# maxjiang93/space_time_pde

Measured on AMD Instinct MI355X. Metric: query-points/sec (fwd+PDE-residual bwd), rb2d 128^3 latent, higher is better.
Workload: dtype f32; 1 GPU; BASELINE configs[1]: latent [1,32,128,128,32], 2^20 query points, RB2 (3 transport + continuity), ImNet nf=32 softplus, L1 losses, backward to ImNet + UNet3d parameters; points=1048576, parallelism=points sharded x1, unet=UNet3d(igres=(32, 128, 128), nf=16, mf=256) fwd+bwd inside the timed step

## Files before the change

include/stpde_hip.h:

```cpp
#ifndef STPDE_HIP_H
#define STPDE_HIP_H

#ifdef __cplusplus
extern "C" {
#endif

#define STPDE_OK 0
#define STPDE_E_BADARG 1
#define STPDE_E_UNSUPPORTED 2
#define STPDE_E_LAUNCH 3

#define STPDE_ACT_TANH 0
#define STPDE_ACT_RELU 1
#define STPDE_ACT_SOFTPLUS 2
#define STPDE_ACT_ELU 3
#define STPDE_ACT_SWISH 4
#define STPDE_ACT_LEAKYRELU 5

#define STPDE_XT 3
#define STPDE_PBAR_SLOTS 64

typedef struct {
  int S1;
  int S2;
  int pair0[6];
  int pair1[6];
  int act;
  float act_param;
  int combo;
  float alpha[6];
} stpde_jet_cfg;

int stpde_version(void);
int stpde_last_error(char* buf, unsigned long n);
#define STPDE_TUNE_CONV3_LDS_OFF 0
#define STPDE_TUNE_CONV3_LDS_MINBLK 1
#define STPDE_TUNE_CONV3_LDS_GX 2
#define STPDE_TUNE_CONV_WGRAD_LDS_GX 3
#define STPDE_TUNE_CONV1_WGRAD_LDS_GX 4
#define STPDE_TUNE_WGRAD_FP32_SWAP 5
#define STPDE_TUNE_COUNT 6
int stpde_tune(const char* name, int value);
int stpde_trace_enable(int on);
long stpde_trace_read(char* buf, unsigned long n);

typedef struct {
  int P, N, B, n0, n1, n2, C;
  int p_base;
  float lo_c[3], hi_c[3], cube[3];
  float alpha[6];
} stpde_gather_desc;
int stpde_lig_gather(const stpde_gather_desc* d, const float* pts, const float* latent, float* X, float* XR,
                     float* coef, int* cell, float* cw , void* stream);

typedef struct {
  int ntiles, KT, MT, first_hidden;
  stpde_jet_cfg cfg;
  int mfma_bf16;
  int packed;
  int det;
} stpde_layer_desc;
int stpde_jet_layer_fwd(const stpde_layer_desc* d, const float* in_pre, const float* X, const float* Wh_pack,
                        const float* Ws_pack, const float* tanc, const float* W0s_pack, const float* tanc0,
                        float* out_pre, const float* cw ,
// ... 10 lines not shown
int stpde_jet_tail_bwd(const stpde_jet_cfg* cfg, int ntiles, int nf16, const float* abar5, const float* const* WhT_pack,
                       const float* const* pre, float* const* abar_out, const float* cw, float* act_param_bar,
                       void* stream);

int stpde_jet_tail_bwd_p(const stpde_jet_cfg* cfg, int ntiles, int nf16, const float* abar5, const float* const* WhT_pack,
                         const float* const* pre, float* const* abar_out, const float* cw, float* act_param_bar, int packed,
                         const void* const* WhT16_pack, void* stream);

int stpde_jet_layer_bwd(const stpde_layer_desc* d, const float* abar_out, const float* WhT_pack, float* in_pre,
                        const float* X, const float* W0s_pack, const float* tanc0, float* abar0, const float* cw,
                        float* act_param_bar, const void* WhT_pack_bf16 ,
                        float* abar0_tan, const float* z0, void* stream);

int stpde_jet_layer_bwd_to(const stpde_layer_desc* d, const float* abar_out, const float* WhT_pack, const float* in_pre,
                           float* abar_in, const float* cw, float* act_param_bar, const void* WhT_pack_bf16, void* stream);

int stpde_jet_wgrad(const stpde_layer_desc* d, int SP, const float* abar_out, const float* in_pre, const float* X,
                    const float* tanc0, float* dW_aug, const float* cw, void* stream);

int stpde_jet_fc1_bwd_supported(const stpde_layer_desc* d);
int stpde_jet_fc1_bwd(const stpde_layer_desc* d, const float* abar1, const void* WhT_pack_bf16, const float* z0,
                      const float* tanc0, const float* cw, const float* X, float* abar0, float* abar0_tan, float* dW_aug,
                      float* act_param_bar, void* stream);

int stpde_lig_reduce_fwd(const stpde_jet_cfg* cfg, int S_mlp, int P, int n_out, const float* out_pre,
                         const float* coef, float* jets, long ldp, void* stream);
int stpde_lig_reduce_bwd(const stpde_jet_cfg* cfg, int S_mlp, int P, int n_out, const float* jets_bar, long ldp,
                         const float* coef, float* abar_out, void* stream);

int stpde_jet_tan0_reduce(int ntiles, int MT, const float* abar0_tan, float* dW_aug, int ldw, int det ,
                          void* stream);

typedef struct {
  int ntiles, nlayers, C, n1, n2;
  int MT[8];
  int SP[8];
  int packed[8];
  int S[8];
} stpde_xbar_desc;
int stpde_lig_xbar_scatter(const stpde_xbar_desc* d, const float* const* abar, const float* const* WsL_pack,
                           const int* cell, float* dlatent, void* stream);
int stpde_lig_xbar_rows(const stpde_xbar_desc* d, const float* const* abar, const float* const* WsL_pack,
                        float* xrows, void* stream);
int stpde_lig_dlatent_reduce(int B, int n0, int n1, int n2, int C, const float* xrows, const int* perm,
                             const int* start, float* dlatent, void* stream);

// ... 23 lines not shown
  float* abar3x;
  float* tan0;
  float* abar0;
  float* abar1x;
  float* abar0x;
  float* xrows;
  int* perm;
  int* start;
  void* sort_tmp;
  unsigned long sort_tmp_bytes;
  float* abar4x;
} stpde_lig_workspace;
#define STPDE_F_STASH 1
#define STPDE_F_VALUE_TILES 2
#define STPDE_F_FUSED_TAIL 4
#define STPDE_F_TAN0_ROWSUM 8
#define STPDE_F_DETERMINISTIC 16
#define STPDE_F_WGRAD 32
#define STPDE_F_WGRAD_FP32 64
#define STPDE_F_PHASE_A 128
#define STPDE_F_PHASE_B 256
#define STPDE_F_NO_FC1_FUSED 512
#define STPDE_F_DET 1024
int stpde_lig_imnet_jet_fwd(const stpde_imnet_plan* plan, const stpde_jet_cfg* cfg_mlp, const stpde_jet_cfg* cfg_out,
                            const stpde_gather_desc* gd, const float* pts, const float* latent,
                            const stpde_lig_workspace* ws, float* jets, long ldp, int flags, void* stream);
int stpde_lig_imnet_jet_bwd(const stpde_imnet_plan* plan, const stpde_jet_cfg* cfg_mlp, const stpde_jet_cfg* cfg_out,
                            const stpde_jet_cfg* cfg_val, const stpde_gather_desc* gd, const stpde_lig_workspace* ws,
                            const float* jets_bar, long ldp, float* dW_flat, float* dlatent, float* act_param_bar,
                            int flags, void* stream);
unsigned long stpde_lig_sort_tmp_bytes(int P, long n_nodes);
int stpde_lig_cell_sort(int P, long n_nodes, const int* cell, int* perm, int* start, void* tmp, unsigned long tmp_bytes,
                        void* stream);

typedef struct {
  int P, N, B, dim, C;
  int n[4];
  float lo_c[4], hi_c[4], cube[4];
} stpde_interp_desc;
int stpde_interp_fwd(const stpde_interp_desc* d, const float* grid, const float* pts, float* out ,
                     float* corner_values , float* weights ,
                     float* x_relative , void* stream);
int stpde_interp_bwd_grid(const stpde_interp_desc* d, const float* pts, const float* out_bar,
                          const float* corner_bar, float* dgrid, void* stream);

typedef struct {
// ... 248 lines not shown
```

space_time_pde_amd/_lib.py:

```python
import ctypes as C
import os
import subprocess
import threading

_HERE = os.path.dirname(os.path.abspath(__file__))
_CSRC = os.path.join(_HERE, "csrc")
LIB_PATH = os.environ.get("STPDE_LIB") or os.path.join(_HERE, "libstpde_hip.so")
_SOURCES = ["jet_layer.hip", "jet_layer_s00.hip", "jet_layer_s03.hip", "jet_layer_s30.hip", "jet_layer_s31.hip", "jet_layer_s32.hip", "jet_layer_s34.hip", "jet_layer_s36.hip", "jet_tail.hip", "jet_wgrad.hip", "jet_wgrad_s00.hip", "jet_wgrad_s30.hip", "jet_wgrad_s31.hip", "jet_wgrad_s32.hip", "jet_wgrad_s34.hip", "jet_wgrad_s36.hip", "jet_fc1_bwd.hip", "lig_gather_reduce.hip", "lig_pipeline.hip", "interp_nd.hip", "conv3d.hip", "conv3d_fused.hip", "optim.hip", "residual.hip", "bn.hip", "resample.hip", "sampler.hip", "sampler_median.hip", "api.cpp"]
_HIPFLAGS = ["--offload-arch=gfx950", "-O3", "-std=c++17", "-fPIC", "-ffp-contract=off", "-munsafe-fp-atomics",
             "--offload-compress"]

ABI_VERSION = 316

ACT_CODES = {"tanh": 0, "relu": 1, "softplus": 2, "elu": 3, "swish": 4, "leakyrelu": 5}
PBAR_SLOTS = 64
XT = 3


class JetCfg(C.Structure):
    _fields_ = [("S1", C.c_int), ("S2", C.c_int), ("pair0", C.c_int * 6), ("pair1", C.c_int * 6),
                ("act", C.c_int), ("act_param", C.c_float), ("combo", C.c_int), ("alpha", C.c_float * 6)]


class GatherDesc(C.Structure):
    _fields_ = [("P", C.c_int), ("N", C.c_int), ("B", C.c_int), ("n0", C.c_int), ("n1", C.c_int), ("n2", C.c_int),
                ("C", C.c_int), ("p_base", C.c_int), ("lo_c", C.c_float * 3), ("hi_c", C.c_float * 3),
                ("cube", C.c_float * 3), ("alpha", C.c_float * 6)]


class GatherNdDesc(C.Structure):
    _fields_ = [("D", C.c_int), ("P", C.c_int), ("N", C.c_int), ("B", C.c_int), ("C", C.c_int), ("p_base", C.c_int),
# ... 6 lines not shown
                ("mfma_bf16", C.c_int), ("packed", C.c_int), ("det", C.c_int)]


class XbarDesc(C.Structure):
    _fields_ = [("ntiles", C.c_int), ("nlayers", C.c_int), ("C", C.c_int), ("n1", C.c_int), ("n2", C.c_int),
                ("MT", C.c_int * 8), ("SP", C.c_int * 8), ("packed", C.c_int * 8), ("S", C.c_int * 8)]


class ImNetPlanDesc(C.Structure):
    _fields_ = [("nlayers", C.c_int), ("cin", C.c_int), ("cout", C.c_int), ("nf16", C.c_int), ("KT", C.c_int * 8),
                ("MT", C.c_int * 8), ("Wh", C.c_void_p * 8), ("WhT", C.c_void_p * 8), ("Ws", C.c_void_p * 8),
                ("WsL", C.c_void_p * 8), ("tanc", C.c_void_p * 8), ("Wh16", C.c_void_p * 8), ("WhT16", C.c_void_p * 8),
                ("mfma_bf16", C.c_int), ("packed_mask", C.c_int), ("dw_off", C.c_long * 8)]


class LigWorkspace(C.Structure):
    _fields_ = [("X", C.c_void_p), ("XR", C.c_void_p), ("coef", C.c_void_p), ("cw", C.c_void_p), ("cell", C.c_void_p),
                ("pre", C.c_void_p * 8), ("abar2x", C.c_void_p), ("abar3x", C.c_void_p), ("tan0", C.c_void_p),
                ("abar0", C.c_void_p), ("abar1x", C.c_void_p), ("abar0x", C.c_void_p), ("xrows", C.c_void_p), ("perm", C.c_void_p), ("start", C.c_void_p),
                ("sort_tmp", C.c_void_p), ("sort_tmp_bytes", C.c_ulong), ("abar4x", C.c_void_p)]


F_STASH, F_VALUE_TILES, F_FUSED_TAIL, F_TAN0_ROWSUM, F_DETERMINISTIC, F_WGRAD, F_WGRAD_FP32 = 1, 2, 4, 8, 16, 32, 64
F_PHASE_A, F_PHASE_B, F_NO_FC1_FUSED, F_DET = 128, 256, 512, 1024
LOSS_DET = 16


class Conv3dDesc(C.Structure):
    _fields_ = [("B", C.c_int), ("T", C.c_int), ("Z", C.c_int), ("X", C.c_int), ("Ci", C.c_int), ("Co", C.c_int),
                ("ksize", C.c_int), ("det", C.c_int), ("mfma_bf16", C.c_int)]


class Conv3dFusedArgs(C.Structure):
    _fields_ = [("d", Conv3dDesc), ("x", C.c_void_p), ("w_pack", C.c_void_p), ("bias", C.c_void_p), ("y", C.c_void_p),
                ("x2", C.c_void_p), ("w2_pack", C.c_void_p), ("y2", C.c_void_p), ("wo2_pack", C.c_void_p),
                ("bias2", C.c_void_p), ("in_sums", C.c_void_p), ("in_gamma", C.c_void_p), ("in_beta", C.c_void_p),
                ("in_running_mean", C.c_void_p), ("in_running_var", C.c_void_p), ("in_stat", C.c_void_p),
                ("out_sums", C.c_void_p), ("m", C.c_void_p), ("m_stat", C.c_void_p), ("m_gamma", C.c_void_p),
                ("m_beta", C.c_void_p), ("m_bsum", C.c_void_p), ("Ci2", C.c_int), ("Co2", C.c_int),
                ("in_eps", C.c_float), ("in_momentum", C.c_float)]


class ResampleDesc(C.Structure):
    _fields_ = [("B", C.c_int), ("T", C.c_int), ("Z", C.c_int), ("X", C.c_int), ("C", C.c_int), ("ft", C.c_int),
                ("fz", C.c_int), ("fx", C.c_int)]


# ... 155 lines not shown
    "stpde_lig_dlatent_reduce_nd": ([C.c_int, C.c_int, C.POINTER(C.c_int), C.c_int, _VP, _VP, _VP, _VP, _VP], C.c_int),
    "stpde_lig_coef_nd": ([C.POINTER(GatherNdDesc), _VP, _VP, _VP], C.c_int),
    "stpde_lig_reduce_nd_jet_fwd": ([C.POINTER(JetCfg), C.c_int, C.c_int, C.c_int, C.c_int, C.c_int, _VP, _VP, _VP, C.c_long,
                                     _VP], C.c_int),
    "stpde_lig_reduce_nd_jet_bwd": ([C.POINTER(JetCfg), C.c_int, C.c_int, C.c_int, C.c_int, C.c_int, _VP, C.c_long, _VP, _VP,
                                     _VP], C.c_int),
    "stpde_jet_wgrad_nd": ([C.POINTER(LayerDesc), C.c_int] + [_VP] * 6 + [C.c_int, _VP], C.c_int),
    "stpde_jet_tan0_reduce_nd": ([C.c_int, C.c_int, _VP, _VP, C.c_int, C.c_int, C.c_int, _VP], C.c_int),
    "stpde_jet_layer_fwd": ([C.POINTER(LayerDesc)] + [_VP] * 12, C.c_int),
    "stpde_jet_layer_bwd": ([C.POINTER(LayerDesc)] + [_VP] * 13, C.c_int),
    "stpde_jet_layer_bwd_to": ([C.POINTER(LayerDesc)] + [_VP] * 8, C.c_int),
    "stpde_jet_tail_fwd": ([C.POINTER(JetCfg), C.c_int, C.c_int, _VP, _VP, C.POINTER(_VP), C.POINTER(_VP), C.POINTER(_VP),
                            C.POINTER(_VP), _VP, _VP], C.c_int),
    "stpde_jet_tail_bwd": ([C.POINTER(JetCfg), C.c_int, C.c_int, _VP, C.POINTER(_VP), C.POINTER(_VP), C.POINTER(_VP), _VP,
                            _VP, _VP], C.c_int),
    "stpde_jet_tail_fwd_p": ([C.POINTER(JetCfg), C.c_int, C.c_int, _VP, _VP, C.POINTER(_VP), C.POINTER(_VP), C.POINTER(_VP),
                              C.POINTER(_VP), _VP, C.c_int, C.POINTER(_VP), _VP], C.c_int),
    "stpde_jet_tail_bwd_p": ([C.POINTER(JetCfg), C.c_int, C.c_int, _VP, C.POINTER(_VP), C.POINTER(_VP), C.POINTER(_VP), _VP,
                              _VP, C.c_int, C.POINTER(_VP), _VP], C.c_int),
    "stpde_jet_tan0_reduce": ([C.c_int, C.c_int, _VP, _VP, C.c_int, C.c_int, _VP], C.c_int),
    "stpde_jet_wgrad": ([C.POINTER(LayerDesc), C.c_int] + [_VP] * 7, C.c_int),
    "stpde_jet_fc1_bwd_supported": ([C.POINTER(LayerDesc)], C.c_int),
    "stpde_jet_fc1_bwd": ([C.POINTER(LayerDesc)] + [_VP] * 11, C.c_int),
    "stpde_lig_reduce_fwd": ([C.POINTER(JetCfg), C.c_int, C.c_int, C.c_int, _VP, _VP, _VP, C.c_long, _VP], C.c_int),
    "stpde_lig_reduce_bwd": ([C.POINTER(JetCfg), C.c_int, C.c_int, C.c_int, _VP, C.c_long, _VP, _VP, _VP], C.c_int),
    "stpde_lig_xbar_scatter": ([C.POINTER(XbarDesc), C.POINTER(_VP), C.POINTER(_VP), _VP, _VP, _VP], C.c_int),
    "stpde_lig_xbar_rows": ([C.POINTER(XbarDesc), C.POINTER(_VP), C.POINTER(_VP), _VP, _VP], C.c_int),
    "stpde_lig_dlatent_reduce": ([C.c_int] * 5 + [_VP] * 5, C.c_int),
    "stpde_lig_imnet_jet_fwd": ([C.POINTER(ImNetPlanDesc), C.POINTER(JetCfg), C.POINTER(JetCfg), C.POINTER(GatherDesc), _VP,
                                 _VP, C.POINTER(LigWorkspace), _VP, C.c_long, C.c_int, _VP], C.c_int),
    "stpde_lig_imnet_jet_bwd": ([C.POINTER(ImNetPlanDesc), C.POINTER(JetCfg), C.POINTER(JetCfg), C.POINTER(JetCfg),
                                 C.POINTER(GatherDesc), C.POINTER(LigWorkspace), _VP, C.c_long, _VP, _VP, _VP, C.c_int, _VP],
                                C.c_int),
    "stpde_lig_sort_tmp_bytes": ([C.c_int, C.c_long], C.c_ulong),
    "stpde_lig_cell_sort": ([C.c_int, C.c_long, _VP, _VP, _VP, _VP, C.c_ulong, _VP], C.c_int),
    "stpde_interp_fwd": ([C.POINTER(InterpDesc)] + [_VP] * 7, C.c_int),
    "stpde_interp_bwd_grid": ([C.POINTER(InterpDesc)] + [_VP] * 5, C.c_int),
    "stpde_conv3d_fwd": ([C.POINTER(Conv3dDesc)] + [_VP] * 5, C.c_int),
    "stpde_conv3d_wgrad": ([C.POINTER(Conv3dDesc)] + [_VP] * 4, C.c_int),
    "stpde_conv3d_wgrad_bias": ([C.POINTER(Conv3dDesc)] + [_VP] * 5, C.c_int),
    "stpde_conv3d_fused": ([C.POINTER(Conv3dFusedArgs), C.POINTER(C.c_int), _VP], C.c_int),
    "stpde_conv3d_wgrad_onload": ([C.POINTER(Conv3dDesc)] + [_VP] * 8, C.c_int),
    "stpde_residual_fwd": ([_VP, C.c_int, C.c_int, C.c_int, C.c_int, _VP, C.c_long, C.c_long, _VP, _VP, _VP], C.c_int),
    "stpde_residual_bwd": ([_VP, C.c_int, C.c_int, C.c_int, C.c_int, _VP, C.c_long, C.c_long, _VP, _VP, _VP, _VP],
                           C.c_int),
    "stpde_residual_coef_fwd": ([_VP, C.c_int, C.c_int, C.c_int, C.c_int, _VP, C.c_long, C.c_long, _VP, _VP,
# ... 46 lines not shown
                    fn.restype = restype
                if h.stpde_version() != ABI_VERSION:
                    raise RuntimeError("libstpde_hip.so at %s has ABI version %d, this package needs %d: rebuild it "
                                       "(python -c 'import __graft_entry__ as g; g.build()')"
                                       % (LIB_PATH, h.stpde_version(), ABI_VERSION))
                _lib = h
    return _lib


_EXC = {1: ValueError, 2: NotImplementedError, 3: RuntimeError}


def check(rc):
    if rc != 0:
        buf = C.create_string_buffer(512)
        lib().stpde_last_error(buf, 512)
        raise _EXC.get(rc, RuntimeError)("libstpde_hip: " + buf.value.decode())


def tune(name, value):
    prev = lib().stpde_tune(name.encode(), int(value))
    if prev < 0:
        raise KeyError(name)
    return prev


class tuned:

    def __init__(self, **kv):
        self.kv, self.prev = kv, {}

    def __enter__(self):
        for k, v in self.kv.items():
            self.prev[k] = tune(k, v)
        return self

    def __exit__(self, *exc):
        for k, v in self.prev.items():
            tune(k, v)
        return False


class dispatch_trace:

    def __enter__(self):
        lib().stpde_trace_enable(1)
        self.kernels = []
# ... 61 lines not shown
```

space_time_pde_amd/csrc/api.cpp:

```cpp
#include <hip/hip_runtime.h>

#include <cstdarg>
#include <cstdio>
#include <cstring>
#include <mutex>
#include <set>
#include <string>

#include "../../include/stpde_hip.h"

static thread_local char g_err[512] = "";

void stpde_set_error(const char* fmt, ...) {
  va_list ap;
  va_start(ap, fmt);
  vsnprintf(g_err, sizeof(g_err), fmt, ap);
  va_end(ap);
}

int stpde_check_launch(const char* what) {
  hipError_t e = hipGetLastError();
  if (e != hipSuccess) {
    stpde_set_error("%s: launch failed: %s", what, hipGetErrorString(e));
    return STPDE_E_LAUNCH;
  }
  return STPDE_OK;
}

extern "C" int stpde_version(void) { return 316; }

#include <atomic>
static const char* const g_tune_names[STPDE_TUNE_COUNT] = {"conv3_lds_off", "conv3_lds_minblk", "conv3_lds_gx", "conv_wgrad_lds_gx",
                                                           "conv1_wgrad_lds_gx", "wgrad_fp32_swap"};
static std::atomic<int> g_tune[STPDE_TUNE_COUNT];
int stpde_tune_get(int key) { return (key >= 0 && key < STPDE_TUNE_COUNT) ? g_tune[key].load(std::memory_order_relaxed) : 0; }
extern "C" int stpde_tune(const char* name, int value) {
  if (!name) return -1;
  for (int k = 0; k < STPDE_TUNE_COUNT; ++k)
    if (!strcmp(name, g_tune_names[k])) return g_tune[k].exchange(value);
  stpde_set_error("stpde_tune: unknown key '%s'", name);
  return -1;
}

extern "C" int stpde_last_error(char* buf, unsigned long n) {
  if (!buf || n == 0) return STPDE_E_BADARG;
  strncpy(buf, g_err, n - 1);
  buf[n - 1] = 0;
  return STPDE_OK;
}

int stpde_trace_on = 0;
static std::mutex g_trace_mu;
static std::set<std::string> g_trace;

void stpde_trace_note(const char* launcher, const char* kernel) {
  std::lock_guard<std::mutex> lk(g_trace_mu);
// ... 21 lines not shown
```

space_time_pde_amd/csrc/lig_pipeline.hip:

```cpp
#include <hipcub/hipcub.hpp>

#include "common.h"

namespace {

struct Seq {
  int rc = STPDE_OK;
  template <class F>
  void operator()(F&& f) {
    if (rc == STPDE_OK) rc = f();
  }
};

bool is_packed(const stpde_imnet_plan* p, int l) { return l >= 0 && ((p->packed_mask >> l) & 1); }

int packed_flags(const stpde_imnet_plan* p, int l, int writes) {
  return ((l >= 2 && is_packed(p, l - 1)) ? 1 : 0) | ((writes >= 0 && is_packed(p, writes)) ? 2 : 0) | (is_packed(p, l) ? 4 : 0);
}

stpde_layer_desc layer_desc(int ntiles, const stpde_imnet_plan* p, int l, const stpde_jet_cfg& cfg, int bf16) {
  stpde_layer_desc d{};
  d.ntiles = ntiles;
  d.KT = p->KT[l];
  d.MT = p->MT[l];
// ... 205 lines not shown
      });
      return;
    }
    seq([&] {
      return stpde_jet_layer_bwd(&d, abar[l], p->WhT[l], l > 1 ? ws->pre[l - 1] : nullptr, ws->X, p->Ws[0], p->tanc[0], abar0,
                                 ws->cw, act_param_bar, w16, (l == 1 && split0) ? ws->tan0 : nullptr, l == 1 ? z0 : nullptr,
                                 stream);
    });
  };
  const bool fc1_fused_on = [&]() -> bool {
    if (!wgrad || !split0 || (flags & STPDE_F_NO_FC1_FUSED)) return false;
    stpde_layer_desc d = layer_desc(nt, p, 1, cfg, p->mfma_bf16 ? p->mfma_bf16 : 0);
    d.packed = packed_flags(p, 1, 0);
    return p->WhT16[1] && stpde_jet_fc1_bwd_supported(&d) != 0 && abar0 != z0;
  }();
  auto fc1_fused_ok = [&]() -> bool { return fc1_fused_on; };
  auto fc1_fused = [&] {
    stpde_layer_desc d = layer_desc(nt, p, 1, cfg, p->mfma_bf16);
    d.packed = packed_flags(p, 1, 0);
    d.det = det;
    seq([&] {
      return stpde_jet_fc1_bwd(&d, abar[1], p->WhT16[1], z0, p->tanc[0], ws->cw, ws->X, abar0, ws->tan0,
                               dW_flat + aw * p->dw_off[1], act_param_bar, stream);
    });
  };
  auto dlatent_part = [&] {
    if (!dlatent) return;
    stpde_xbar_desc xd{};
    xd.ntiles = nt;
    xd.nlayers = 5;
    xd.C = p->cin;
    xd.n1 = gd->n1;
    xd.n2 = gd->n2;
    const float* ab[5];
    const float* wt[5];
    for (int l = 0; l < 5; ++l) {
      xd.MT[l] = p->MT[l];
      xd.SP[l] = l == 0 ? (split0 ? 1 : SP0) : S;
      xd.packed[l] = is_packed(p, l) ? 1 : 0;
      xd.S[l] = l == 0 ? 1 : S;
      ab[l] = l == 0 ? abar0 : abar[l];
      wt[l] = p->WsL[l];
    }
    if (!(flags & STPDE_F_DETERMINISTIC)) {
      seq([&] { return stpde_lig_xbar_scatter(&xd, ab, wt, ws->cell, dlatent, stream); });
    } else {
// ... 10 lines not shown
    if (phaseA) {
      seq([&] { return stpde_lig_reduce_bwd(cfg_out, S, gd->P, p->cout, jets_bar, ldp, ws->coef, ws->pre[NL - 1], stream); });
      if (wgrad) wgrad_l(5);
      tail_bwd();
      dgrad_l(2);
      if (fc1_fused_ok())
        fc1_fused();
      else
        dgrad_l(1);
      dlatent_part();
    }
    if (phaseB && wgrad) {
      for (int l = 4; l >= (fc1_fused_ok() ? 2 : 1); --l) wgrad_l(l);
      wgrad_0();
    }
    return seq.rc;
  }
  seq([&] { return stpde_lig_reduce_bwd(cfg_out, S, gd->P, p->cout, jets_bar, ldp, ws->coef, ws->pre[NL - 1], stream); });
  for (int l = NL - 1; l >= 1; --l) {
    if (l == 1 && fc1_fused_ok()) {
      fc1_fused();
      continue;
    }
    if (wgrad) wgrad_l(l);
    if (tail && l >= 3) {
      if (l == 5) tail_bwd();
      continue;
    }
    dgrad_l(l);
  }
  if (wgrad) wgrad_0();
  dlatent_part();
  return seq.rc;
}
```

space_time_pde_amd/lig_jet.py:

```python
import ctypes as C
import dataclasses
import math
import os
import threading

import numpy as np
import torch

from . import _lib
from ._lib import XT, GatherDesc, GatherNdDesc, ImNetPlanDesc, JetCfg, LayerDesc, LigWorkspace, XbarDesc, check, ptr, stream_ptr

_FRAG = 256
MAX_LATENT_CHANNELS = 16 * (XT - 1) + 4 - 3 - 1
MAX_AUG_FEATURES = 16 * (XT - 1) + 4
ND_VALUE_DIMS = (1, 2, 4)
ND_TRAIN_MAX_CHANNELS = 32

nd_backward = os.getenv("STPDE_ND_BACKWARD", "0").strip().lower() not in ("", "0", "false", "no", "off")


def set_nd_backward(on):
    global nd_backward
    prev, nd_backward = nd_backward, bool(on)
    return prev
# ... 300 lines not shown
    S_out: int
    pairs: list
    bf16: bool
    nsplit: int
    packed_mask: int
    B: int
    N: int
    grid_shape: tuple
    lo_c: list
    hi_c: list
    cube: list
    P_pad: int
    budget: object
    recompute: bool
    chunk: int
    need_grad: bool
    det: bool
    det_dlatent: bool
    value_tiles: bool
    tan0_rowsum: bool
    wgrad_split: bool
    fused_tail: bool
    fc1_fused: bool
    nd_backward: bool
    nd_jets: bool
    nd_jet_backward: bool
    pipeline: bool
    tail: bool
    SP0: int
    split0: bool
    mult: int

    @classmethod
    def make(cls, plan, act, act_param, first, pairs, combo, precision, grid_shape, box, budget=None, B=1, N=0,
             chunk_points=None, need_grad=True):
        precision = precision or mlp_precision
        if precision not in ("fp32", "bf16", "fp32x3"):
            raise ValueError("mlp precision must be 'fp32', 'bf16' or 'fp32x3'")
        dim = plan.dim
        if dim != 3 and precision == "bf16":
            raise NotImplementedError("dim = %d value queries run with fp32 or fp32x3 operands" % dim)
        cfg_out, S_out, ppairs = make_cfg(act, act_param, first, list(pairs), combo)
        cfg, S = cfg_out, S_out
        if act in ("relu", "leakyrelu") and ppairs:
            cfg, S, _ = make_cfg(act, act_param, True, [])
        tail = _tail_applies(fused_tail, plan.nf, cfg, cfg_out.combo)
        packed = (precision == "bf16" and packed_stash and plan.nf == 32 and S <= 6 and tail and cfg.S1 == 3 and tan0_rowsum)
        mult = (8 if S == 1 else 2) if dim == 3 else 4 * (16 >> dim)
        chunk_points = chunk_points or (DEFAULT_CHUNK if dim == 3 else (DEFAULT_CHUNK // 2) * (16 >> dim))
        P, SP0 = B * N, 1 + cfg.S1
        return cls(plan=plan, cfg=cfg, cfg_out=cfg_out, cfg_val=make_cfg(act, act_param, False, [])[0], S=S, S_out=S_out,
                   pairs=ppairs, bf16=precision in ("bf16", "fp32x3"), nsplit=3 if precision == "fp32x3" else 1,
                   packed_mask=31 if packed else 0, B=B, N=N, grid_shape=tuple(grid_shape), lo_c=box[0], hi_c=box[1],
                   cube=box[2], P_pad=P + ((-P) % mult if dim == 3 else 0),
                   budget=budget if budget is not None else memory_budget, recompute=bool(force_recompute),
                   chunk=max(mult, chunk_points // mult * mult), need_grad=bool(need_grad), det=bool(_lib.deterministic),
                   det_dlatent=bool(deterministic_dlatent), value_tiles=bool(value_tiles), tan0_rowsum=bool(tan0_rowsum),
                   wgrad_split=bool(wgrad_split), fused_tail=bool(fused_tail), fc1_fused=fc1_fused_enabled(),
                   nd_backward=bool(nd_backward), nd_jets=bool(nd_jets),
                   nd_jet_backward=bool(nd_jets and nd_jet_backward),
                   pipeline=bool(use_pipeline and profile is None and dim == 3),
                   tail=tail, SP0=SP0, split0=bool(SP0 == 4 and tan0_rowsum), mult=mult)

    def plan_chunk(self, points):
        object.__setattr__(self, "chunk", points)


def _AW(call):
    return 2 * _lib.DET_K if call.det else 1


def _dw_slice(call, dw_flat, l):
    off, mp, ka = call.plan.dw_off[l]
    return dw_flat[_AW(call) * off:_AW(call) * (off + mp * ka)]


def _layer_desc(call, ntiles, lay, cfg, first_hidden, bf16=0, packed=0):
    d = LayerDesc()
    d.ntiles, d.KT, d.MT, d.first_hidden, d.cfg = ntiles, lay["KT"], lay["MT"], int(first_hidden), cfg
    d.mfma_bf16 = int(bf16)
    d.packed = int(packed)
# ... 41 lines not shown
        if packs16:
            d.Wh16[l], d.WhT16[l] = _dp(packs16.get((l, "Wh"))), _dp(packs16.get((l, "WhT")))
        d.dw_off[l] = plan.dw_off[l][0]
    d.mfma_bf16 = call.nsplit if packs16 else 0
    d.packed_mask = call.packed_mask
    return d


def _gather_desc(call, latent, Pc, p0):
    gd = GatherDesc()
    gd.P, gd.N, gd.B = Pc, call.N, call.B
    gd.n0, gd.n1, gd.n2, gd.C = latent.shape[1], latent.shape[2], latent.shape[3], latent.shape[4]
    for k in range(3):
        gd.lo_c[k], gd.hi_c[k], gd.cube[k] = call.lo_c[k], call.hi_c[k], call.cube[k]
    gd.p_base = p0
    for k in range(6):
        gd.alpha[k] = call.cfg_out.alpha[k]
    return gd


def _flags(call, need_grad, need_wgrad=True):
    bits = ((need_grad, _lib.F_STASH), (call.value_tiles, _lib.F_VALUE_TILES), (call.fused_tail, _lib.F_FUSED_TAIL),
            (call.tan0_rowsum, _lib.F_TAN0_ROWSUM), (call.det_dlatent, _lib.F_DETERMINISTIC), (need_wgrad, _lib.F_WGRAD),
            (not call.wgrad_split, _lib.F_WGRAD_FP32), (not call.fc1_fused, _lib.F_NO_FC1_FUSED), (call.det, _lib.F_DET))
    return sum(bit for on, bit in bits if on)


def nd_tiles(P, dim):
    tp = 16 >> dim
    return (-(-P // tp) + 3) // 4 * 4


_LAYER_BUFS = tuple("buf%d" % l for l in range(1, 6))
_FWD_ORDER = {True: ("X", "cw", "coef", "cell") + _LAYER_BUFS + ("z0",),
              False: ("X", "cw", "roww", "coef", "cell", "buf1", "z0") + _LAYER_BUFS[1:]}
_BWD_ORDER = {True: ("abar2x", "abar3x", "abar1x", "abar4x", "abar0x", "tan0", "abar0"),
              False: ("abar0", "abar0x", "tan0", "abar1x", "abar4x", "abar3x", "abar2x")}
_DTYPES = dict(cell=torch.int32, perm=torch.int32, start=torch.int32, sort_tmp=torch.uint8)
SORT_TMP_PLAN_BYTES = 24


def _table(order, size):
    return [(k, size[k], _DTYPES.get(k, torch.float32)) for k in order if size.get(k) is not None]


def _chunk_tiles(call, Pc):
    return nd_tiles(Pc, call.plan.dim) if call.plan.dim != 3 else Pc // 2
# ... 186 lines not shown
    elif nd:
        with _timed("reduce_nd_bwd"):
            check(L.stpde_lig_reduce_nd_bwd(plan.dim, Pc, nt, plan.cout, C.c_void_p(jets_bar.data_ptr() + 4 * p0),
                                            jets_bar.shape[2], ptr(saved["roww"]), ptr(bufs[5]), st))
    else:
        with _timed("reduce_bwd"):
            check(L.stpde_lig_reduce_bwd(C.byref(call.cfg_out), S, Pc, plan.cout, C.c_void_p(jets_bar.data_ptr() + 4 * p0),
                                         jets_bar.shape[2], ptr(coef), ptr(bufs[5]), st))
    MT0 = plan.layers[0]["MT"]
    adj = _alloc(_backward_buffers(call, Pc), dev)
    abar0, tan0 = adj.get("abar0x", adj.get("abar0", z0)), adj.get("tan0")
    abar = {l: adj.get("abar%dx" % l, bufs[l]) for l in range(1, 6)}
    for l in range(5, 0, -1):
        lay = plan.layers[l]
        w16 = packs16.get((l, "WhT")) if packs16 else None
        d = _layer_desc(call, nt, lay, cfg, l == 1, call.nsplit if w16 is not None else 0, _pk(call, l, l - 1))
        dwg = _layer_desc(call, nt, lay, cfg, l == 1, (call.nsplit if call.wgrad_split or call.nsplit == 1 else 0)
                          if (w16 is not None and lay["MT"] >= 8) else 0, _pk(call, l, -1) & 5)
        if (l == 1 and need_wgrad and split0 and w16 is not None and abar0 is not z0
                and call.fc1_fused and L.stpde_jet_fc1_bwd_supported(C.byref(d))):
            with _timed("layer1_bwd"):
                check(L.stpde_jet_fc1_bwd(C.byref(d), ptr(abar[1]), ptr(w16), ptr(z0), ptr(pv(packs, 0, "tanc")), ptr(cw),
                                          ptr(X), ptr(abar0), ptr(tan0), ptr(_dw_slice(call, dw_flat, 1)), ptr(pbar), st))
            continue
        if need_wgrad:
            with _timed("layer%d_wgrad" % l):
                check(wgrad(dwg, S, abar[l], bufs[l - 1] if l > 1 else saved["z0"], pv(packs, 0, "tanc"),
                            _dw_slice(call, dw_flat, l), cw))
        if call.tail and l >= 3:
            if l == 5:
                arr = lambda ts: (C.c_void_p * 3)(*[t.data_ptr() for t in ts])
                pk_tail = (call.packed_mask >> 2) & 1
                w16s = (C.c_void_p * 3)(packs16[(3, "WhT")].data_ptr(), packs16[(4, "WhT")].data_ptr(), None) \
                    if pk_tail else None
                with _timed("tail_dgrad"):
                    check(L.stpde_jet_tail_bwd_p(C.byref(cfg), nt, plan.nf // 16, ptr(bufs[5]),
                                                 arr([pv(packs, k, "WhT") for k in (3, 4, 5)]),
                                                 arr([bufs[2], bufs[3], bufs[4]]), arr([abar[2], abar[3], abar[4]]),
                                                 ptr(cw), ptr(pbar), 3 if pk_tail else 0, w16s, st))
            continue
        if l > 1 and abar[l - 1] is not bufs[l - 1]:
            with _timed("layer%d_dgrad" % l):
                check(L.stpde_jet_layer_bwd_to(C.byref(d), ptr(abar[l]), ptr(pv(packs, l, "WhT")), ptr(bufs[l - 1]),
                                               ptr(abar[l - 1]), ptr(cw), ptr(pbar), ptr(w16), st))
            continue
        with _timed("layer%d_dgrad" % l):
# ... 236 lines not shown
        if type(module) is cls:
            if name == "softplus" and (module.beta != 1 or module.threshold != 20):
                return None
            if name == "elu" and module.alpha != 1.0:
                return None
            if name == "leakyrelu" and module.negative_slope != 0.01:
                return None
            return name, 0.0
    return None


deterministic_dlatent = True
value_tiles = True
tan0_rowsum = True
wgrad_split = True
packed_stash = True
fused_tail = True

force_recompute = False


def fc1_fused_enabled():
    return os.environ.get("STPDE_FC1_FUSED", "1") != "0"

DEFAULT_CHUNK = 1 << 20

mlp_precision = os.environ.get("STPDE_MLP_PRECISION", "fp32")


def set_mlp_precision(precision):
    global mlp_precision
    if precision not in ("fp32", "bf16", "fp32x3"):
        raise ValueError("mlp precision must be 'fp32', 'bf16' or 'fp32x3'")
    prev, mlp_precision = mlp_precision, precision
    return prev


_ND_VALUE_ONLY = "dim = %d queries run in HIP as value-only forward passes (no coordinate derivatives)"


def lig_jets(imnet, latent_grid, query_pts, xmin, xmax, first=True, pairs=(), chunk_points=None, combo=None,
             precision=None, memory_budget=None):
    if not (latent_grid.is_cuda and query_pts.is_cuda):
        raise RuntimeError("the HIP jet path needs CUDA/HIP tensors (no CPU fallback)")
    dim = imnet.dim
    wants_jets = bool(first or len(pairs) or combo)
# ... 72 lines not shown
```

space_time_pde_amd/train_step.py:

```python
import os

import torch
import torch.distributed as dist
import torch.nn.functional as F

from . import _lib, lig_jet
from .local_implicit_grid import query_local_implicit_grid


last_collectives = []


class _SumGradAcrossRanks(torch.autograd.Function):

    @staticmethod
    def forward(ctx, x):
        return x.view_as(x)

    @staticmethod
    def backward(ctx, g):
        hooks = lig_jet.sync_hooks
        done = hooks.get("dlatent_done") if hooks else None
        if done is None:
            g = g.contiguous()
# ... 52 lines not shown
            and not (b is not None and b.requires_grad):
        return _LossSumHip.apply(a, b, _LOSS_KIND[loss_type])
    return _LOSS_SUMS[loss_type](a, torch.zeros_like(a) if b is None else b)


def _coefficient_leaves(pde_layer):
    vals = getattr(pde_layer, "params", None) or {}
    return [vals[s.name] for s in getattr(pde_layer, "param_vars", ()) if s.name in vals and vals[s.name].requires_grad
            and vals[s.name].is_leaf]


def sharded_step(unet, imnet, pde_layer, input_grid, point_coord, point_value, n_points_global, alpha_reg=1.0,
                 alpha_pde=1.0, loss_type="l1", xmin=0.0, xmax=1.0, distributed=None, sync_unet_grads=False):
    if distributed is None:
        distributed = dist.is_available() and dist.is_initialized() and dist.get_world_size() > 1
    if loss_type not in _LOSS_SUMS:
        raise KeyError(loss_type)
    if distributed and any(t.requires_grad and not t.is_leaf for t in (getattr(pde_layer, "params", None) or {}).values()):
        raise NotImplementedError("sharded_step(distributed=True): a grad-requiring equation coefficient must be a leaf tensor "
                                  "(the gradient of a leaf behind it would not be summed over ranks)")
    prev_deferred = getattr(unet, "deferred_weight_grads", None)
    if prev_deferred is not None:
        unet.deferred_weight_grads = os.environ.get("STPDE_UNET_DEFERRED", "1") != "0"
    try:
        return _sharded_step(unet, imnet, pde_layer, input_grid, point_coord, point_value, n_points_global, alpha_reg,
                             alpha_pde, loss_type, xmin, xmax, distributed, sync_unet_grads)
    finally:
        if prev_deferred is not None:
            unet.deferred_weight_grads = prev_deferred


def _sharded_step(unet, imnet, pde_layer, input_grid, point_coord, point_value, n_points_global, alpha_reg, alpha_pde,
                  loss_type, xmin, xmax, distributed, sync_unet_grads):
    latent_grid = unet(input_grid).permute(0, 2, 3, 4, 1)
    if distributed:
        latent_grid = _SumGradAcrossRanks.apply(latent_grid)
    pde_layer.update_forward_method(lambda pts: query_local_implicit_grid(imnet, latent_grid, pts, xmin, xmax))
    overlap_sync = distributed and os.environ.get("STPDE_OVERLAP_SYNC", "1") != "0"
    lig_jet.expect_two_phase = bool(overlap_sync)
    try:
        pred, residues = pde_layer(point_coord, return_residue=True)
    finally:
        lig_jet.expect_two_phase = False
    b = point_coord.shape[0]
    reg = loss_sum(pred, point_value, loss_type) / (b * n_points_global * pred.shape[-1])
    res = list(residues.values())
    base = res[0]._base if all(r._base is not None and r._base is res[0]._base for r in res) else None
    stack = base if (base is not None and base.numel() == sum(r.numel() for r in res)) else torch.stack(res, dim=0)
    pde = loss_sum(stack, None, loss_type) / (len(res) * b * n_points_global)
    loss = alpha_reg * reg + alpha_pde * pde
# ... 178 lines not shown
```

Before: 2.523 million query-points/s.

## Fuse second hidden layer backward data-grad and weight-grad into one kernel

Adds a fused HIP kernel for the layer-2 ImNet jet backward that computes the adjoint into layer 1 (through the activation jet) and the weight gradient, including the raw-input and tangent row-sum columns, in a single pass over the tiles. The goal is to avoid reading abar2 and pre1 twice across separate backward-to and wgrad launches, and to save a launch. It is switched on by default inside sharded_step for the fp32 unpacked configuration and can be disabled through a tune knob. In exchange it adds heavy LDS use and an MFMA schedule that relies on many sched_barrier pins.

```diff
diff --git a/include/stpde_hip.h b/include/stpde_hip.h
--- a/include/stpde_hip.h
+++ b/include/stpde_hip.h
@@ -39,7 +39,8 @@
 #define STPDE_TUNE_CONV_WGRAD_LDS_GX 3
 #define STPDE_TUNE_CONV1_WGRAD_LDS_GX 4
 #define STPDE_TUNE_WGRAD_FP32_SWAP 5
-#define STPDE_TUNE_COUNT 6
+#define STPDE_TUNE_FC2_BWD_FUSED 6
+#define STPDE_TUNE_COUNT 7
 int stpde_tune(const char* name, int value);
 int stpde_trace_enable(int on);
 long stpde_trace_read(char* buf, unsigned long n);
@@ -96,6 +97,10 @@
 int stpde_jet_fc1_bwd(const stpde_layer_desc* d, const float* abar1, const void* WhT_pack_bf16, const float* z0,
                       const float* tanc0, const float* cw, const float* X, float* abar0, float* abar0_tan, float* dW_aug,
                       float* act_param_bar, void* stream);
+
+int stpde_jet_fc2_bwd_supported(const stpde_layer_desc* d);
+int stpde_jet_fc2_bwd(const stpde_layer_desc* d, const float* abar2, const float* WhT_pack, const float* pre1, const float* X,
+                      const float* cw, float* abar1, float* dW_aug, float* act_param_bar, void* stream);
 
 int stpde_lig_reduce_fwd(const stpde_jet_cfg* cfg, int S_mlp, int P, int n_out, const float* out_pre,
                          const float* coef, float* jets, long ldp, void* stream);
@@ -165,6 +170,7 @@
 #define STPDE_F_PHASE_B 256
 #define STPDE_F_NO_FC1_FUSED 512
 #define STPDE_F_DET 1024
+#define STPDE_F_FC2_FUSED 2048
 int stpde_lig_imnet_jet_fwd(const stpde_imnet_plan* plan, const stpde_jet_cfg* cfg_mlp, const stpde_jet_cfg* cfg_out,
                             const stpde_gather_desc* gd, const float* pts, const float* latent,
                             const stpde_lig_workspace* ws, float* jets, long ldp, int flags, void* stream);
diff --git a/space_time_pde_amd/_lib.py b/space_time_pde_amd/_lib.py
--- a/space_time_pde_amd/_lib.py
+++ b/space_time_pde_amd/_lib.py
@@ -6,7 +6,7 @@
 _HERE = os.path.dirname(os.path.abspath(__file__))
 _CSRC = os.path.join(_HERE, "csrc")
 LIB_PATH = os.environ.get("STPDE_LIB") or os.path.join(_HERE, "libstpde_hip.so")
-_SOURCES = ["jet_layer.hip", "jet_layer_s00.hip", "jet_layer_s03.hip", "jet_layer_s30.hip", "jet_layer_s31.hip", "jet_layer_s32.hip", "jet_layer_s34.hip", "jet_layer_s36.hip", "jet_tail.hip", "jet_wgrad.hip", "jet_wgrad_s00.hip", "jet_wgrad_s30.hip", "jet_wgrad_s31.hip", "jet_wgrad_s32.hip", "jet_wgrad_s34.hip", "jet_wgrad_s36.hip", "jet_fc1_bwd.hip", "lig_gather_reduce.hip", "lig_pipeline.hip", "interp_nd.hip", "conv3d.hip", "conv3d_fused.hip", "optim.hip", "residual.hip", "bn.hip", "resample.hip", "sampler.hip", "sampler_median.hip", "api.cpp"]
+_SOURCES = ["jet_layer.hip", "jet_layer_s00.hip", "jet_layer_s03.hip", "jet_layer_s30.hip", "jet_layer_s31.hip", "jet_layer_s32.hip", "jet_layer_s34.hip", "jet_layer_s36.hip", "jet_tail.hip", "jet_wgrad.hip", "jet_wgrad_s00.hip", "jet_wgrad_s30.hip", "jet_wgrad_s31.hip", "jet_wgrad_s32.hip", "jet_wgrad_s34.hip", "jet_wgrad_s36.hip", "jet_fc1_bwd.hip", "jet_fc2_bwd.hip", "lig_gather_reduce.hip", "lig_pipeline.hip", "interp_nd.hip", "conv3d.hip", "conv3d_fused.hip", "optim.hip", "residual.hip", "bn.hip", "resample.hip", "sampler.hip", "sampler_median.hip", "api.cpp"]
 _HIPFLAGS = ["--offload-arch=gfx950", "-O3", "-std=c++17", "-fPIC", "-ffp-contract=off", "-munsafe-fp-atomics",
              "--offload-compress"]
 
@@ -59,7 +59,7 @@
 
 
 F_STASH, F_VALUE_TILES, F_FUSED_TAIL, F_TAN0_ROWSUM, F_DETERMINISTIC, F_WGRAD, F_WGRAD_FP32 = 1, 2, 4, 8, 16, 32, 64
-F_PHASE_A, F_PHASE_B, F_NO_FC1_FUSED, F_DET = 128, 256, 512, 1024
+F_PHASE_A, F_PHASE_B, F_NO_FC1_FUSED, F_DET, F_FC2_FUSED = 128, 256, 512, 1024, 2048
 LOSS_DET = 16
 
 
@@ -261,6 +261,8 @@
     "stpde_jet_wgrad": ([C.POINTER(LayerDesc), C.c_int] + [_VP] * 7, C.c_int),
     "stpde_jet_fc1_bwd_supported": ([C.POINTER(LayerDesc)], C.c_int),
     "stpde_jet_fc1_bwd": ([C.POINTER(LayerDesc)] + [_VP] * 11, C.c_int),
+    "stpde_jet_fc2_bwd_supported": ([C.POINTER(LayerDesc)], C.c_int),
+    "stpde_jet_fc2_bwd": ([C.POINTER(LayerDesc)] + [_VP] * 9, C.c_int),
     "stpde_lig_reduce_fwd": ([C.POINTER(JetCfg), C.c_int, C.c_int, C.c_int, _VP, _VP, _VP, C.c_long, _VP], C.c_int),
     "stpde_lig_reduce_bwd": ([C.POINTER(JetCfg), C.c_int, C.c_int, C.c_int, _VP, C.c_long, _VP, _VP, _VP], C.c_int),
     "stpde_lig_xbar_scatter": ([C.POINTER(XbarDesc), C.POINTER(_VP), C.POINTER(_VP), _VP, _VP, _VP], C.c_int),
@@ -353,7 +355,15 @@
     prev = lib().stpde_tune(name.encode(), int(value))
     if prev < 0:
         raise KeyError(name)
+    _tune_values[name] = int(value)
     return prev
+
+
+_tune_values = {}
+
+
+def tune_value(name):
+    return _tune_values.get(name, 0)
 
 
 class tuned:
diff --git a/space_time_pde_amd/csrc/api.cpp b/space_time_pde_amd/csrc/api.cpp
--- a/space_time_pde_amd/csrc/api.cpp
+++ b/space_time_pde_amd/csrc/api.cpp
@@ -31,7 +31,7 @@
 
 #include <atomic>
 static const char* const g_tune_names[STPDE_TUNE_COUNT] = {"conv3_lds_off", "conv3_lds_minblk", "conv3_lds_gx", "conv_wgrad_lds_gx",
-                                                           "conv1_wgrad_lds_gx", "wgrad_fp32_swap"};
+                                                           "conv1_wgrad_lds_gx", "wgrad_fp32_swap", "fc2_bwd_fused"};
 static std::atomic<int> g_tune[STPDE_TUNE_COUNT];
 int stpde_tune_get(int key) { return (key >= 0 && key < STPDE_TUNE_COUNT) ? g_tune[key].load(std::memory_order_relaxed) : 0; }
 extern "C" int stpde_tune(const char* name, int value) {
diff --git a/space_time_pde_amd/csrc/jet_fc2_bwd.hip b/space_time_pde_amd/csrc/jet_fc2_bwd.hip
--- /dev/null
+++ b/space_time_pde_amd/csrc/jet_fc2_bwd.hip
@@ -0,0 +1,261 @@
+#include "jet_layer_impl.h"
+#include "jet_wgrad_impl.h"
+
+#define FC2F_BARRIER()                                     \
+  do {                                                     \
+    asm volatile("s_waitcnt lgkmcnt(0)" ::: "memory");     \
+    __builtin_amdgcn_s_barrier();                          \
+    asm volatile("" ::: "memory");                         \
+  } while (0)
+
+template <int S1, int S2, int ACT>
+__global__ __launch_bounds__(512, 2) void k_fc2_bwd_fused(WgradArgs a, LayerArgs la) {
+  constexpr int S = 1 + S1 + S2, NWV = 8, KTT = 2 * NWV, MCW = NWV, KW = 2;
+  constexpr int TP = 24, TBLK = 16 * TP;
+  constexpr int PIN_MFMA_DSR = 0x2 | 0x4 | 0x10 | 0x20 | 0x40 | 0x200;
+  constexpr bool EARLYP = ACT != STPDE_ACT_SWISH;
+  constexpr int NTW = (MCW + (NWV - XT) - 1) / (NWV - XT);
+  static_assert(S1 == 3 && XT == 3, "tangent streams and three raw-input tiles expected");
+  __shared__ __attribute__((aligned(16))) float pshare[S][MCW][TBLK];
+  __shared__ __attribute__((aligned(16))) float ppriv[NWV][2][TBLK];
+  __shared__ __attribute__((aligned(16))) float pflat[S][MCW][256];
+  __shared__ __attribute__((aligned(16))) float xacc[XT][MCW][256];
+  const int lane = threadIdx.x & 63;
+  const int wv = __builtin_amdgcn_readfirstlane(threadIdx.x >> 6);
+  const int lo = lane * 4;
+  const int g = lane >> 4, c = lane & 15;
+
+  f32x4 acc[MCW][KW];
+#pragma unroll
+  for (int mi = 0; mi < MCW; ++mi) {
+#pragma unroll
+    for (int k = 0; k < KW; ++k) acc[mi][k] = f32x4{0.f, 0.f, 0.f, 0.f};
+    if (wv < XT) st4(&xacc[wv][mi][lo], f32x4{0.f, 0.f, 0.f, 0.f});
+  }
+  float acct[3][NTW];
+#pragma unroll
+  for (int d = 0; d < 3; ++d)
+#pragma unroll
+    for (int q = 0; q < NTW; ++q) acct[d][q] = 0.f;
+  float pacc = 0.f;
+  int flip = 0;
+  auto transpose = [&](f32x4 v) -> f32x4 {
+    float* patch = ppriv[wv][flip];
+    flip ^= 1;
+    lds_put_T<TP>(patch, lane, v);
+    __builtin_amdgcn_wave_barrier();
+    const f32x4 r = lds_get_R<TP>(patch, lane);
+    __builtin_amdgcn_wave_barrier();
+    return r;
+  };
+
+  f32x4 praw[S], qraw[S];
+  auto ldb = [&](const float* buf, int t, int NB, int st, int blk) -> f32x4 {
+    return ld4(buf + (((size_t)t * S + st) * NB + blk) * 256 + (unsigned)lo);
+  };
+  auto load_p = [&](int t) {
+#pragma unroll
+    for (int st = 0; st < S; ++st) praw[st] = ldb(a.P, t, MCW, st, wv);
+  };
+  auto load_qk = [&](int t, int k) {
+#pragma unroll
+    for (int st = 0; st < S; ++st) qraw[st] = ldb(a.Q, t, KTT, st, KW * wv + k);
+  };
+  constexpr int MTD = KTT, KTD = MCW;
+  f32x4 wr[2];
+  auto load_w = [&](int f) {
+    const int k = (f / KTD) % KW, kt = f % KTD;
+    wr[f & 1] = ld4(la.Wp + (size_t)((kt * MTD + KW * wv + k) * 256) + (unsigned)lo);
+  };
+  if ((int)blockIdx.x < a.ntiles) {
+    load_p(blockIdx.x);
+    load_qk(blockIdx.x, 0);
+    load_w(0);
+  }
+#pragma unroll 1
+  for (int tile = blockIdx.x; tile < a.ntiles; tile += gridDim.x) {
+    const int tnext = tile + (int)gridDim.x < a.ntiles ? tile + (int)gridDim.x : tile;
+    float cq[6];
+    load_cq<S2>(a.cw, tile * 2 + (c >> 3), cq);
+#pragma unroll
+    for (int st = 0; st < S; ++st) {
+      lds_put_T<TP>(&pshare[st][wv][0], lane, praw[st]);
+      st4(&pflat[st][wv][lo], praw[st]);
+    }
+    f32x4 xcur = f32x4{0.f, 0.f, 0.f, 0.f};
+    if (wv < XT) xcur = ld4(a.X + ((size_t)tile * XT + wv) * 256 + (unsigned)lo);
+    FC2F_BARRIER();
+#pragma unroll
+    for (int k = 0; k < KW; ++k) {
+      f32x4 gacc[S];
+#pragma unroll
+      for (int st = 0; st < S; ++st) gacc[st] = f32x4{0.f, 0.f, 0.f, 0.f};
+      {
+        f32x4 Bc = ld4(&pflat[0][0][lo]);
+#pragma unroll
+        for (int kt = 0; kt < KTD; ++kt) {
+          const int f = k * KTD + kt;
+          const f32x4 w = wr[f & 1];
+          load_w(f + 1);
+#pragma unroll
+          for (int st = 0; st < S; ++st) {
+            f32x4 Bn = Bc;
+            if (st + 1 < S) Bn = ld4(&pflat[st + 1][kt][lo]);
+            else if (kt + 1 < KTD) Bn = ld4(&pflat[0][kt + 1][lo]);
+            __builtin_amdgcn_sched_barrier(PIN_MFMA_DSR);
+#pragma unroll
+            for (int r = 0; r < 4; ++r) gacc[st] = mfma4(w[r], Bc[r], gacc[st]);
+            __builtin_amdgcn_sched_barrier(PIN_MFMA_DSR);
+            Bc = Bn;
+          }
+        }
+      }
+      __builtin_amdgcn_sched_barrier(0);
+      {
+        f32x4 H[S];
+        act_jet_fwd<S1, S2, ACT>(a.cfg, qraw, H, cq);
+#pragma unroll
+        for (int st = 0; st < S; ++st) {
+          const f32x4 hr = transpose(H[st]);
+          f32x4 pc = lds_get_R<TP>(&pshare[st][0][0], lane);
+#pragma unroll
+          for (int mi = 0; mi < MCW; ++mi) {
+            f32x4 pn = pc;
+            if (mi + 1 < MCW) pn = lds_get_R<TP>(&pshare[st][mi + 1][0], lane);
+            __builtin_amdgcn_sched_barrier(0);
+#pragma unroll
+            for (int r = 0; r < 4; ++r) acc[mi][k] = mfma4(pc[r], hr[r], acc[mi][k]);
+            pc = pn;
+          }
+        }
+      }
+      __builtin_amdgcn_sched_barrier(0);
+      if (EARLYP && k + 1 == KW) load_p(tnext);
+      __builtin_amdgcn_sched_barrier(0);
+      layer_epilogue<S1, S2, EPI_ADJ, ACT, 0>(la, tile, KW * wv + k, MTD, lane, gacc, nullptr, cq, pacc, nullptr, qraw);
+      __builtin_amdgcn_sched_barrier(0);
+      if (k + 1 < KW) load_qk(tile, k + 1);
+      else {
+        load_qk(tnext, 0);
+        if (!EARLYP) load_p(tnext);
+      }
+    }
+    if (wv < XT) {
+      const f32x4 xrr = transpose(xcur);
+#pragma unroll
+      for (int mi = 0; mi < MCW; ++mi) {
+        const f32x4 p0 = lds_get_R<TP>(&pshare[0][mi][0], lane);
+        f32x4 ax = ld4(&xacc[wv][mi][lo]);
+#pragma unroll
+        for (int r = 0; r < 4; ++r) ax = mfma4(p0[r], xrr[r], ax);
+        st4(&xacc[wv][mi][lo], ax);
+      }
+    } else {
+#pragma unroll
+      for (int d = 0; d < 3; ++d)
+#pragma unroll
+        for (int q = 0; q < NTW; ++q) {
+          const int mi = q * (NWV - XT) + wv - XT;
+          if (mi >= MCW) continue;
+          const f32x4 pd = lds_get_R<TP>(&pshare[1 + d][mi][0], lane);
+          acct[d][q] += (pd[0] + pd[1]) + (pd[2] + pd[3]);
+        }
+    }
+    FC2F_BARRIER();
+  }
+  const int ldw = 16 * (KTT + XT);
+#pragma unroll
+  for (int mi = 0; mi < MCW; ++mi) {
+#pragma unroll
+    for (int k = 0; k <= KW; ++k) {
+      if (k == KW && wv >= XT) continue;
+      const int col = k < KW ? 16 * (KW * wv + k) : 16 * (KTT + wv);
+      const f32x4 v = k < KW ? acc[mi][k < KW ? k : 0] : ld4(&xacc[wv < XT ? wv : 0][mi][lo]);
+#pragma unroll
+      for (int r = 0; r < 4; ++r) acc_add_f32(a.dW, (size_t)(16 * mi + 4 * g + r) * ldw + col + c, v[r], a.det);
+    }
+  }
+  if (wv >= XT) {
+#pragma unroll
+    for (int q = 0; q < NTW; ++q)
+#pragma unroll
+      for (int d = 0; d < 3; ++d) {
+        const int mi = q * (NWV - XT) + wv - XT;
+        if (mi >= MCW) continue;
+        float v = acct[d][q];
+        v += __shfl_xor(v, 16, 64);
+        v += __shfl_xor(v, 32, 64);
+        if (g == 0 && d < a.ncoord) acc_add_f32(a.dW, (size_t)(16 * mi + c) * ldw + 16 * KTT + d, v, a.det);
+      }
+  }
+  flush_pbar<EPI_ADJ, ACT>(la, pacc, lane);
+}
+
+template <int S1, int S2, int ACT>
+static int launch_fc2_fused(const WgradArgs& a, const LayerArgs& la, hipStream_t stream) {
+  int gx = 256;
+  if (gx > a.ntiles) gx = a.ntiles;
+  STPDE_LAUNCH((k_fc2_bwd_fused<S1, S2, ACT>), dim3(gx), dim3(512), 0, stream, a, la);
+  return stpde_check_launch("k_fc2_bwd_fused");
+}
+
+template <int S1, int S2>
+static int launch_fc2_fused_act(const WgradArgs& a, const LayerArgs& la, hipStream_t stream) {
+  switch (a.cfg.act) {
+    case STPDE_ACT_TANH: return launch_fc2_fused<S1, S2, STPDE_ACT_TANH>(a, la, stream);
+    case STPDE_ACT_RELU: return launch_fc2_fused<S1, S2, STPDE_ACT_RELU>(a, la, stream);
+    case STPDE_ACT_SOFTPLUS: return launch_fc2_fused<S1, S2, STPDE_ACT_SOFTPLUS>(a, la, stream);
+    case STPDE_ACT_ELU: return launch_fc2_fused<S1, S2, STPDE_ACT_ELU>(a, la, stream);
+    case STPDE_ACT_LEAKYRELU: return launch_fc2_fused<S1, S2, STPDE_ACT_LEAKYRELU>(a, la, stream);
+    default: return launch_fc2_fused<S1, S2, STPDE_ACT_SWISH>(a, la, stream);
+  }
+}
+
+extern "C" int stpde_jet_fc2_bwd_supported(const stpde_layer_desc* d) {
+  if (!d) return 0;
+  const bool combo = d->cfg.S2 == 1 && d->cfg.combo;
+  return !d->first_hidden && d->mfma_bf16 == 0 && d->packed == 0 && d->KT == 16 && d->MT == 8 && XT == 3 && d->cfg.S1 == 3 &&
+         (d->cfg.S2 == 0 || combo) && d->cfg.act >= 0 && d->cfg.act <= 5;
+}
+
+extern "C" int stpde_jet_fc2_bwd(const stpde_layer_desc* d, const float* abar2, const float* WhT_pack, const float* pre1,
+                                 const float* X, const float* cw, float* abar1, float* dW_aug, float* act_param_bar,
+                                 void* stream) {
+  if (!stpde_jet_fc2_bwd_supported(d)) {
+    stpde_set_error("jet_fc2_bwd: exact fp32, unpacked buffers only (second hidden layer of the reference width: KT = 16, MT = 8, "
+                    "S1 = 3, S2 = 0 or the combined stream)");
+    return STPDE_E_UNSUPPORTED;
+  }
+  if (d->ntiles <= 0 || !abar2 || !WhT_pack || !pre1 || !X || !abar1 || !dW_aug || (d->cfg.S2 && !cw) || abar1 == abar2) {
+    stpde_set_error("jet_fc2_bwd: bad argument");
+    return STPDE_E_BADARG;
+  }
+  const int S = 1 + d->cfg.S1 + d->cfg.S2;
+  WgradArgs a{};
+  a.P = abar2;
+  a.Q = pre1;
+  a.X = X;
+  a.dW = dW_aug;
+  a.cw = cw;
+  a.SP = S;
+  a.KT = d->KT;
+  a.MT = d->MT;
+  a.ntiles = d->ntiles;
+  a.cfg = d->cfg;
+  a.det = d->det;
+  a.ncoord = 3;
+  LayerArgs la{};
+  la.Bin = abar2;
+  la.Wp = WhT_pack;
+  la.Out = abar1;
+  la.Pre = pre1;
+  la.cw = cw;
+  la.pbar = act_param_bar;
+  la.nsplit = 1;
+  la.KT = d->MT;
+  la.MT = d->KT;
+  la.ntiles = d->ntiles;
+  la.cfg = d->cfg;
+  if (d->cfg.S2 == 1) return launch_fc2_fused_act<3, 1>(a, la, (hipStream_t)stream);
+  return launch_fc2_fused_act<3, 0>(a, la, (hipStream_t)stream);
+}
diff --git a/space_time_pde_amd/csrc/lig_pipeline.hip b/space_time_pde_amd/csrc/lig_pipeline.hip
--- a/space_time_pde_amd/csrc/lig_pipeline.hip
+++ b/space_time_pde_amd/csrc/lig_pipeline.hip
@@ -251,6 +251,20 @@
     seq([&] {
       return stpde_jet_fc1_bwd(&d, abar[1], p->WhT16[1], z0, p->tanc[0], ws->cw, ws->X, abar0, ws->tan0,
                                dW_flat + aw * p->dw_off[1], act_param_bar, stream);
+    });
+  };
+  const bool fc2_fused_on = [&]() -> bool {
+    if (!wgrad || dfirst || !(flags & STPDE_F_FC2_FUSED) || stpde_tune_get(STPDE_TUNE_FC2_BWD_FUSED) == 2) return false;
+    stpde_layer_desc d = layer_desc(nt, p, 2, cfg, p->mfma_bf16);
+    d.packed = packed_flags(p, 2, 1);
+    return stpde_jet_fc2_bwd_supported(&d) != 0;
+  }();
+  auto fc2_fused = [&] {
+    stpde_layer_desc d = layer_desc(nt, p, 2, cfg, 0);
+    d.det = det;
+    seq([&] {
+      return stpde_jet_fc2_bwd(&d, abar[2], p->WhT[2], ws->pre[1], ws->X, ws->cw, abar[1], dW_flat + aw * p->dw_off[2],
+                               act_param_bar, stream);
     });
   };
   auto dlatent_part = [&] {
@@ -307,6 +321,10 @@
       fc1_fused();
       continue;
     }
+    if (l == 2 && fc2_fused_on) {
+      fc2_fused();
+      continue;
+    }
     if (wgrad) wgrad_l(l);
     if (tail && l >= 3) {
       if (l == 5) tail_bwd();
diff --git a/space_time_pde_amd/lig_jet.py b/space_time_pde_amd/lig_jet.py
--- a/space_time_pde_amd/lig_jet.py
+++ b/space_time_pde_amd/lig_jet.py
@@ -346,6 +346,7 @@
     wgrad_split: bool
     fused_tail: bool
     fc1_fused: bool
+    fc2_fused: bool
     nd_backward: bool
     nd_jets: bool
     nd_jet_backward: bool
@@ -381,6 +382,7 @@
                    chunk=max(mult, chunk_points // mult * mult), need_grad=bool(need_grad), det=bool(_lib.deterministic),
                    det_dlatent=bool(deterministic_dlatent), value_tiles=bool(value_tiles), tan0_rowsum=bool(tan0_rowsum),
                    wgrad_split=bool(wgrad_split), fused_tail=bool(fused_tail), fc1_fused=fc1_fused_enabled(),
+                   fc2_fused=fc2_fused_enabled(),
                    nd_backward=bool(nd_backward), nd_jets=bool(nd_jets),
                    nd_jet_backward=bool(nd_jets and nd_jet_backward),
                    pipeline=bool(use_pipeline and profile is None and dim == 3),
@@ -468,7 +470,8 @@
 def _flags(call, need_grad, need_wgrad=True):
     bits = ((need_grad, _lib.F_STASH), (call.value_tiles, _lib.F_VALUE_TILES), (call.fused_tail, _lib.F_FUSED_TAIL),
             (call.tan0_rowsum, _lib.F_TAN0_ROWSUM), (call.det_dlatent, _lib.F_DETERMINISTIC), (need_wgrad, _lib.F_WGRAD),
-            (not call.wgrad_split, _lib.F_WGRAD_FP32), (not call.fc1_fused, _lib.F_NO_FC1_FUSED), (call.det, _lib.F_DET))
+            (not call.wgrad_split, _lib.F_WGRAD_FP32), (not call.fc1_fused, _lib.F_NO_FC1_FUSED), (call.det, _lib.F_DET),
+            (call.fc2_fused, _lib.F_FC2_FUSED))
     return sum(bit for on, bit in bits if on)
 
 
@@ -701,6 +704,12 @@
             with _timed("layer1_bwd"):
                 check(L.stpde_jet_fc1_bwd(C.byref(d), ptr(abar[1]), ptr(w16), ptr(z0), ptr(pv(packs, 0, "tanc")), ptr(cw),
                                           ptr(X), ptr(abar0), ptr(tan0), ptr(_dw_slice(call, dw_flat, 1)), ptr(pbar), st))
+            continue
+        if (l == 2 and need_wgrad and call.fc2_fused and not nd and w16 is None
+                and L.stpde_jet_fc2_bwd_supported(C.byref(dwg))):
+            with _timed("layer2_bwd"):
+                check(L.stpde_jet_fc2_bwd(C.byref(dwg), ptr(abar[2]), ptr(pv(packs, 2, "WhT")), ptr(bufs[1]), ptr(X), ptr(cw),
+                                          ptr(abar[1]), ptr(_dw_slice(call, dw_flat, 2)), ptr(pbar), st))
             continue
         if need_wgrad:
             with _timed("layer%d_wgrad" % l):
@@ -983,6 +992,14 @@
 
 def fc1_fused_enabled():
     return os.environ.get("STPDE_FC1_FUSED", "1") != "0"
+
+
+fc2_fused = None
+
+
+def fc2_fused_enabled():
+    return bool(fc2_fused) and _lib.tune_value("fc2_bwd_fused") != 2
+
 
 DEFAULT_CHUNK = 1 << 20
 
diff --git a/space_time_pde_amd/train_step.py b/space_time_pde_amd/train_step.py
--- a/space_time_pde_amd/train_step.py
+++ b/space_time_pde_amd/train_step.py
@@ -98,10 +98,14 @@
     prev_deferred = getattr(unet, "deferred_weight_grads", None)
     if prev_deferred is not None:
         unet.deferred_weight_grads = os.environ.get("STPDE_UNET_DEFERRED", "1") != "0"
+    prev_fc2 = lig_jet.fc2_fused
+    if prev_fc2 is None:
+        lig_jet.fc2_fused = True
     try:
         return _sharded_step(unet, imnet, pde_layer, input_grid, point_coord, point_value, n_points_global, alpha_reg,
                              alpha_pde, loss_type, xmin, xmax, distributed, sync_unet_grads)
     finally:
+        lig_jet.fc2_fused = prev_fc2
         if prev_deferred is not None:
             unet.deferred_weight_grads = prev_deferred
 
```

After: 2.569 million query-points/s, median of 6. 1.8% higher.
